# hvasbath/beat

Measured on AMD Instinct MI355X. Metric: SMC chain-steps/s (FFI seismic gfstacking 400 patches x 64 targets x 4096 samples), higher is better.
Workload: dtype f64; 1 GPU; BASELINE configs[2]: FFI seismic gfstacking, 400 patches x 64 targets x 4096 samples, library (64,400,3,25,4096) f64 = 62.9 GB in HBM, nearest_neighbor, covariance scalar; population SURVEY 8(d): nucleation U over the 20x20 fault, time 0; chains_per_gpu=512, global_chains=512, parallelism=chains sharded over 1 GPU(s), library replicated

## Files before the change

beat_amd/csrc/ctx.cpp:

```cpp
#include "ctx.hpp"

#include <cstdlib>

namespace beatamd {

static thread_local char g_err[1024] = "";

void set_error(const char *fmt, ...)
{
    va_list ap;
    va_start(ap, fmt);
    vsnprintf(g_err, sizeof(g_err), fmt, ap);
    va_end(ap);
}

int DevBuf::reserve(size_t bytes)
{
    if (bytes <= cap) return BEATAMD_OK;
    size_t want = bytes + bytes / 4;
    if (p) {
        BA_HIP(hipDeviceSynchronize());
        BA_HIP(hipFree(p));
        p = nullptr;
        cap = 0;
// ... 127 lines not shown
{
    BA_HIP(hipStreamSynchronize(stream));
    int st = 0;
    BA_HIP(hipMemcpy(&st, d_status, sizeof(int), hipMemcpyDeviceToHost));
    if (st) {
        BA_HIP(hipMemset(d_status, 0, sizeof(int)));
        if (st & ST_INDEX_OOB) {
            set_error("index out of bounds of the GF library "
                      "(duration/starttime outside the library grid)");
            return BEATAMD_EINDEX;
        }
        if (st & ST_BAD_HYPO) {
            set_error("nucleation index outside the patch grid");
            return BEATAMD_EINVAL;
        }
        if (st & ST_BAD_COV) {
            set_error("Sample covariances contains Inf or NaN! Please try reducing the upper and lower bounds "
                      "of hyper parameters!");
            return BEATAMD_EBADCOV;
        }
        if (st & ST_NOT_PSD) {
            set_error("Matrix is not positive definite");
            return BEATAMD_ENOTPSD;
        }
        if (st & ST_LINE_NONFINITE) {
            set_error("trace_density: a sample or an extent that is not finite (or xmax <= xmin)");
            return BEATAMD_EINVAL;
        }
        if (st & ST_LINE_OOB) {
            set_error("Line endpoint outside of given grid (an index above the last cell, or below -32768)");
            return BEATAMD_EOUTSIDE;
        }
        if (st & ST_BAD_SCALE) {
            set_error("PoissonProposal: a step width outside (0, 500] (or NaN): the draws of that parameter are NaN");
            return BEATAMD_EINVAL;
        }
    }
    return BEATAMD_OK;
}

namespace beatamd {

void GfKnobs::read_env()
{
    auto rd = [](const char *name) { const char *e = getenv(name); return e ? atoi(e) : KNOB_UNSET; };
    gf_kernel = rd("BEATAMD_GF_KERNEL"); gs_cg = rd("BEATAMD_GS_CG"); gs_ws = rd("BEATAMD_GS_WS"); gs_dma = rd("BEATAMD_GS_DMA");
    gs_nt = rd("BEATAMD_GS_NT"); ws_map = rd("BEATAMD_WS_MAP"); gs_pair = rd("BEATAMD_GS_PAIR"); gs_nthint = rd("BEATAMD_GS_NTHINT");
    gs_order = rd("BEATAMD_GS_ORDER"); gs_fit = rd("BEATAMD_GS_FIT"); gs_win = rd("BEATAMD_GS_WIN"); gf_tinv = rd("BEATAMD_GF_TINV");
    gs_tune = rd("BEATAMD_GS_TUNE"); gf_order = rd("BEATAMD_GF_ORDER"); gf_cgroup = rd("BEATAMD_GF_CGROUP"); gs_ml = rd("BEATAMD_GS_ML");
    gc_global = rd("BEATAMD_GC_GLOBAL"); gc_sort = rd("BEATAMD_GC_SORT"); gc_keys = rd("BEATAMD_GC_KEYS"); gc_bands = rd("BEATAMD_GC_BANDS"); gr_cap = rd("BEATAMD_GR_CAP");
    gr_pass_alloc = rd("BEATAMD_GR_PASS_ALLOC"); gr_var = rd("BEATAMD_GR_VAR"); sweep_v1 = rd("BEATAMD_SWEEP_V1"); qf_band = rd("BEATAMD_QF_BAND"); qf_fuse = rd("BEATAMD_QF_FUSE"); gf_split = rd("BEATAMD_GF_SPLIT"); gm_wave = rd("BEATAMD_GM_WAVE");
    skip_parked = rd("BEATAMD_SKIP_PARKED");
    td_strip = rd("BEATAMD_TD_STRIP");
}

const GfKnobs &gf_knobs(beatamd_ctx *ctx)
{
    if (ctx->knobs_live) ctx->knobs.read_env();
    return ctx->knobs;
}

}

extern "C" {

const char *beatamd_last_error(void) { return g_err; }

int beatamd_version(void) { return BEATAMD_VERSION; }

int beatamd_ctx_create(int device, beatamd_ctx **out)
{
    BA_CHECK(out != nullptr, BEATAMD_EINVAL, "ctx_create: out is NULL");
    int ndev = 0;
    hipError_t e = hipGetDeviceCount(&ndev);
    if (e != hipSuccess || ndev == 0) {
        (void)hipGetLastError();
        set_error("no HIP device available (%s)", hipGetErrorString(e));
        return BEATAMD_EHIP;
    }
    BA_CHECK(device >= 0 && device < ndev, BEATAMD_EINVAL, "device %d out of range [0,%d)", device,
             ndev);
    BA_HIP(hipSetDevice(device));
    beatamd_ctx *c = new beatamd_ctx();
    c->device = device;
    BA_HIP(hipStreamCreateWithFlags(&c->own_stream, hipStreamNonBlocking));
    c->stream = c->own_stream;
    BA_HIP(hipMalloc((void **)&c->d_status, sizeof(int)));
    BA_HIP(hipMemset(c->d_status, 0, sizeof(int)));
    hipDeviceProp_t prop;
    BA_HIP(hipGetDeviceProperties(&prop, device));
    c->num_cu = prop.multiProcessorCount;
    c->scratch_bufs.resize(SL_COUNT);
    c->knobs.read_env();
    {
        const char *live = getenv("BEATAMD_KNOBS_LIVE");
        c->knobs_live = live && atoi(live) != 0;
    }
    *out = c;
    return BEATAMD_OK;
}

int beatamd_ctx_reload_knobs(beatamd_ctx *c)
{
    BA_CHECK(c != nullptr, BEATAMD_EINVAL, "ctx_reload_knobs: NULL context");
    c->knobs.read_env();
    return BEATAMD_OK;
}

int beatamd_ctx_destroy(beatamd_ctx *c)
{
    if (!c) return BEATAMD_OK;
    (void)hipSetDevice(c->device);
    (void)hipStreamSynchronize(c->stream);
    c->models.clear();
    c->hypers.clear();
    c->wsets.clear();
    c->laps.clear();
    c->geolibs.clear();
    c->seislibs.clear();
    for (auto &s : c->scratch_bufs) s.release();
    for (auto &kv : c->timers)
        for (auto &pr : kv.second.pending) {
            (void)hipEventDestroy(pr.first);
            (void)hipEventDestroy(pr.second);
        }
    for (auto e : c->event_pool) (void)hipEventDestroy(e);
    if (c->d_status) (void)hipFree(c->d_status);
    if (c->h_umax) (void)hipHostFree(c->h_umax);
    if (c->umax_event) (void)hipEventDestroy(c->umax_event);
    if (c->own_stream) (void)hipStreamDestroy(c->own_stream);
    delete c;
    return BEATAMD_OK;
}

int beatamd_ctx_set_stream(beatamd_ctx *c, void *s)
{
    BA_CHECK(c, BEATAMD_EINVAL, "ctx is NULL");
    BA_HIP(hipSetDevice(c->device));
    c->stream = (hipStream_t)s;
    return BEATAMD_OK;
}

int beatamd_ctx_use_own_stream(beatamd_ctx *c)
{
    BA_CHECK(c, BEATAMD_EINVAL, "ctx is NULL");
    c->stream = c->own_stream;
    return BEATAMD_OK;
}

int beatamd_ctx_set_step_counter(beatamd_ctx *c, uint32_t *device_counter)
{
    BA_CHECK(c != nullptr, BEATAMD_EINVAL, "ctx is NULL");
    BA_CHECK(device_counter == nullptr || is_device_ptr(device_counter), BEATAMD_EINVAL,
             "ctx_set_step_counter: the counter must live in device memory");
    c->step_dev = device_counter;
    return BEATAMD_OK;
}

int beatamd_ctx_synchronize(beatamd_ctx *c)
{
    BA_CHECK(c, BEATAMD_EINVAL, "ctx is NULL");
    BA_HIP(hipSetDevice(c->device));
    return c->check_status();
}

int beatamd_ctx_enable_timing(beatamd_ctx *c, int on)
{
    BA_CHECK(c, BEATAMD_EINVAL, "ctx is NULL");
    c->timing = on != 0;
    return BEATAMD_OK;
}

static int drain_timer(beatamd_ctx *c, KTimer &t)
{
    for (auto &pr : t.pending) {
        BA_HIP(hipEventSynchronize(pr.second));
        float ms = 0.f;
        BA_HIP(hipEventElapsedTime(&ms, pr.first, pr.second));
        t.total_ms += ms;
        t.n += 1;
        c->event_pool.push_back(pr.first);
        c->event_pool.push_back(pr.second);
// ... 33 lines not shown
```

beat_amd/csrc/ctx.hpp:

```cpp
#pragma once
#include <hip/hip_runtime.h>

#include <cstdarg>
#include <cstdint>
#include <cstdio>
#include <cstring>
#include <map>
#include <memory>
#include <string>
#include <vector>

#include "../../include/beat_amd.h"

struct beatamd_ctx;

namespace beatamd {

void set_error(const char *fmt, ...);

#define BA_HIP(expr)                                                                         \
    do {                                                                                     \
        hipError_t e_ = (expr);                                                              \
        if (e_ != hipSuccess) {                                                              \
            beatamd::set_error("%s:%d: %s -> %s", __FILE__, __LINE__, #expr,                 \
// ... 148 lines not shown
    std::vector<int64_t> sizes;
    std::vector<int32_t> wsets;
    DevMem<int64_t> hp_off;
    bool corr_set = false;
    GeoCorr corr;
    DevMem<GeoCorrTerm> corr_terms;
    DevMem<double> corr_basis;
};

struct GeomSources {
    int nsrc = 0;
    DevMem<int32_t> kind;
    DevMem<int64_t> poff;
    DevMem<double> pfix;
    DevMem<double> east, north, los;
    int64_t Nobs = 0;
    double nu = 0.25;
};

struct FfiModel {
    beatamd_ffi_layout layout;
    int32_t nsub = 0;
    std::vector<int32_t> ndip, nstrike, patch_off;
    std::vector<double> patch_size;
    int64_t P = 0;
    DevMem<int32_t> d_ndip, d_nstrike, d_patch_off;
    DevMem<double> d_patch_size;
    std::vector<Wavemap> wavemaps;
    bool has_geo = false;
    Geodetic geo;
    bool geo_is_geometry = false;
    GeomSources geom;
    int32_t lap = -1;
    int64_t nllk() const;
    bool obs_quads_valid = false;
    std::vector<double> obs_quads;
    DevMem<double> d_obs_quads;
};

struct HyperModel {
    int64_t nterm = 0, nh = 0;
    DevMem<double> M, slog;
    DevMem<int32_t> kind, hp_index;
    int32_t ngroups = 0, group_end[8] = {0, 0, 0, 0, 0, 0, 0, 0};
};

constexpr int KNOB_UNSET = -2147483647;
struct GfKnobs {
    int gf_kernel = KNOB_UNSET, gs_cg = KNOB_UNSET, gs_ws = KNOB_UNSET, gs_dma = KNOB_UNSET, gs_nt = KNOB_UNSET,
        ws_map = KNOB_UNSET, gs_pair = KNOB_UNSET, gs_nthint = KNOB_UNSET, gs_order = KNOB_UNSET, gs_fit = KNOB_UNSET,
        gs_win = KNOB_UNSET, gf_tinv = KNOB_UNSET, gs_tune = KNOB_UNSET, gf_order = KNOB_UNSET, gf_cgroup = KNOB_UNSET,
        gs_ml = KNOB_UNSET, gc_global = KNOB_UNSET, gc_sort = KNOB_UNSET, gc_keys = KNOB_UNSET, gc_bands = KNOB_UNSET, gr_cap = KNOB_UNSET,
        gr_pass_alloc = KNOB_UNSET, gr_var = KNOB_UNSET, sweep_v1 = KNOB_UNSET, qf_band = KNOB_UNSET, qf_fuse = KNOB_UNSET, gf_split = KNOB_UNSET, gm_wave = KNOB_UNSET,
        skip_parked = KNOB_UNSET, td_strip = KNOB_UNSET;
    void read_env();
    static int get(int v, int dflt) { return v == KNOB_UNSET ? dflt : v; }
    static bool is(int v, int x) { return v != KNOB_UNSET && v == x; }
    static bool set(int v) { return v != KNOB_UNSET; }
};

struct KTimer {
    double total_ms = 0;
    int64_t n = 0;
    std::vector<std::pair<hipEvent_t, hipEvent_t>> pending;
};

}

struct beatamd_ctx {
    int device = 0;
    hipStream_t stream = nullptr, own_stream = nullptr;
    bool timing = false;
    std::map<std::string, beatamd::KTimer> timers;
    std::vector<hipEvent_t> event_pool;
    int *d_status = nullptr;
    std::vector<beatamd::DevBuf> scratch_bufs;
    std::vector<std::unique_ptr<beatamd::SeisStore>> seislibs;
    std::vector<std::unique_ptr<beatamd::GeoLib>> geolibs;
    std::vector<std::unique_ptr<beatamd::WeightSet>> wsets;
    std::vector<std::unique_ptr<beatamd::Laplacian>> laps;
    std::vector<std::unique_ptr<beatamd::FfiModel>> models;
    std::vector<std::unique_ptr<beatamd::HyperModel>> hypers;
    int num_cu = 256;
    char last_gf_kernel[96] = "";
    int64_t gs_ngtp = 0, gs_N = 0;
    double gs_trep = 1;
    int gs_nvar = 1;
    bool gs_has_passes = false;
    char gf_plan[384] = "";
    bool gf_band_fused = false;
    char gf_tune_log[512] = "";
    uint32_t *h_umax = nullptr;
    hipEvent_t umax_event = nullptr;
    bool umax_pending = false;
    int umax_hist = -1, umax_hist_cg = 0;
    std::map<std::vector<int64_t>, std::pair<int, int>> gs_tuned;
    int gs_cg = 0;
    beatamd::GfKnobs knobs;
    bool knobs_live = false;
    uint32_t *step_dev = nullptr;

    int get_scratch(int slot, size_t bytes, void **out);
    template <class T>
    int scratch(int slot, size_t n, T **out)
    {
        void *raw = nullptr;
        const int rc = get_scratch(slot, n * sizeof(T), &raw);
        *out = static_cast<T *>(raw);
        return rc;
    }
    hipEvent_t get_event();
    void time_begin(const char *name);
    void time_end(const char *name);
    int check_status();
};

namespace beatamd {

bool is_device_ptr(const void *p);
const GfKnobs &gf_knobs(beatamd_ctx *ctx);

enum Slot : int {
    SL_IN0 = 0, SL_IN1, SL_IN2, SL_IN3, SL_IN4, SL_IN5, SL_IN6, SL_IN7,
    SL_OUT0, SL_OUT1, SL_OUT2, SL_OUT3,
    SL_ROWOFF, SL_WEIGHTS, SL_ST0, SL_RESID, SL_PARTIAL, SL_PARTIAL2, SL_QUAD, SL_MU, SL_SLIPS,
    SL_QPROP, SL_LPROP, SL_MISC, SL_GS_UROWS, SL_GS_UCOUNT, SL_GS_SLOT, SL_GS_W, SL_GS_UMAX, SL_GS_USLOT,
    SL_CHAINBAD, SL_Z, SL_ROWSCALE, SL_CUM, SL_STAGE2, SL_WHITEN,
    SL_CHOL_A, SL_CHOL_X, SL_CHOL_D, SL_CHOL_T, SL_CHOL_L,
    SL_GC_ORDER, SL_GS_ORDER, SL_GC_STREAM, SL_GC_HDR, SL_GC_META, SL_DELTA, SL_LOGU, SL_EDGES, SL_TSLOT, SL_SPLIT, SL_WS_PACK, SL_COUNT
};
constexpr int SL_NIN = SL_OUT0 - SL_IN0, SL_NOUT = SL_ROWOFF - SL_OUT0;

class Staging {
    beatamd_ctx *ctx;
    int nin = 0, nout = 0, nback = 0;
    struct { void *host, *dev; size_t bytes; } back[SL_NOUT];
    int in_bytes(const void *p, size_t bytes, const void **dev);
    int out_bytes(void *p, size_t bytes, void **dev, bool preload);

public:
    explicit Staging(beatamd_ctx *c) : ctx(c) {}
    template <class T>
    int in(const T *p, size_t n, const T **dev)
    {
        const void *d = nullptr;
        BA_TRY(in_bytes(p, n * sizeof(T), &d));
        *dev = static_cast<const T *>(d);
        return BEATAMD_OK;
// ... 21 lines not shown
```

beat_amd/csrc/gfshared.hip:

```cpp
#include "kernels.hpp"

namespace beatamd {

constexpr int GS_NT_MAX = 64;
constexpr int GS_NTHINT_DEFAULT = 1;
constexpr int GS_WS_DEFAULT = 1;

struct GroupTabArgs {
    int nrow, nvar, CG;
    int64_t C, T, P, DS;
    const uint32_t *rowoff;
    const double *fac;
    ChainVec slips[4];
    int ucap, ustride;
    uint32_t *urows;
    uint32_t *uent;
    int nissue;
    int windowed;
    int depth;
    uint32_t *ucount;
    uint32_t *umax;
    uint16_t *slot;
    double *w;
    int64_t w_var_stride;
// ... 1141 lines not shown
            gs_store_syn<GS_NT>(a.out + (c * a.T + t) * N + n0, acc, nvalid);
        }
        return;
    }
    __builtin_amdgcn_s_barrier();
    if (tid < GS_NT) xbuf[tid] = (tid < nvalid) ? a.data[t * N + n0 + tid] : 0.0;
    __builtin_amdgcn_fence(__ATOMIC_RELEASE, "workgroup");
    __builtin_amdgcn_s_barrier();
    __builtin_amdgcn_fence(__ATOMIC_ACQUIRE, "workgroup");
    if (MODE == GF_RESID_STORE) {
        gs_resid_store<GS_NT>(a.out + (c * a.T + t) * N + n0, acc, xbuf, live, nvalid);
    } else {
        const double q = gs_misfit_scalar<GS_NT>(a.wscalar[t], acc, xbuf, nvalid);
        if (live) a.partial[(c * a.T + t) * a.ntile + tile] = q;
    }
}


template <int WAVES, int NROW, int MODE>
static int launch_shared_one(dim3 grid, size_t lds, hipStream_t s, const GsArgs &a)
{
    void (*kern)(GsArgs) = nullptr;
    if constexpr (WAVES == 16) {
        kern = k_gfstack_dma<WAVES, NROW, MODE, 32, 1>;
    } else if (a.f32pair) {
        kern = k_gfstack_dmaf<WAVES, NROW, MODE>;
    } else {
        kern = (a.dma == 2 && a.nt == 32) ? k_gfstack_dma<WAVES, NROW, MODE, 32, 1>
             : (a.dma == 2) ? k_gfstack_dma<WAVES, NROW, MODE, 64, 1>
                            : k_gfstack_dma<WAVES, NROW, MODE, 64, 0>;
    }
    if (lds > 64 * 1024)
        BA_HIP(hipFuncSetAttribute((const void *)kern, hipFuncAttributeMaxDynamicSharedMemorySize, (int)lds));
    hipLaunchKernelGGL(kern, grid, dim3(WAVES * 64), lds, s, a);
    return BEATAMD_OK;
}

template <int WAVES, int NROW>
static int launch_shared_mode(int mode, dim3 grid, size_t lds, hipStream_t s, const GsArgs &a)
{
    if (mode == GF_STORE_SYN) return launch_shared_one<WAVES, NROW, GF_STORE_SYN>(grid, lds, s, a);
    if (mode == GF_RESID_SCALAR) return launch_shared_one<WAVES, NROW, GF_RESID_SCALAR>(grid, lds, s, a);
    return launch_shared_one<WAVES, NROW, GF_RESID_STORE>(grid, lds, s, a);
}

template <int WAVES>
static int launch_shared_nrow(int nrow, int mode, dim3 grid, size_t lds, hipStream_t s,
                              const GsArgs &a)
{
    if (nrow == 1) return launch_shared_mode<WAVES, 1>(mode, grid, lds, s, a);
    return launch_shared_mode<WAVES, 4>(mode, grid, lds, s, a);
}

static int launch_ws(int mode, dim3 grid, size_t lds, hipStream_t s, const GsArgs &a, int pair)
{
    void (*kern)(GsArgs);
#define BA_WS_PICK(NAME, ...)                                                                          \
    (mode == GF_STORE_SYN ? NAME<__VA_ARGS__ GF_STORE_SYN, 3, 1>                                      \
     : mode == GF_RESID_SCALAR ? NAME<__VA_ARGS__ GF_RESID_SCALAR, 3, 1> : NAME<__VA_ARGS__ GF_RESID_STORE, 3, 1>)
#define BA_WS_PICK0(NAME, ...)                                                                         \
    (mode == GF_STORE_SYN ? NAME<__VA_ARGS__ GF_STORE_SYN, 3, 0>                                      \
     : mode == GF_RESID_SCALAR ? NAME<__VA_ARGS__ GF_RESID_SCALAR, 3, 0> : NAME<__VA_ARGS__ GF_RESID_STORE, 3, 0>)
    if (pair == 1) kern = a.nthint ? BA_WS_PICK(k_gfstack_wsp, 1,) : BA_WS_PICK0(k_gfstack_wsp, 1,);
    else if (pair == 2) kern = a.nthint ? BA_WS_PICK(k_gfstack_wsp, 0,) : BA_WS_PICK0(k_gfstack_wsp, 0,);
    else if (mode == GF_RESID_BAND1) kern = a.nthint ? k_gfstack_ws<1, GF_RESID_BAND1, 3, 1> : k_gfstack_ws<1, GF_RESID_BAND1, 3, 0>;
    else kern = a.nthint ? BA_WS_PICK(k_gfstack_ws, 1,) : BA_WS_PICK0(k_gfstack_ws, 1,);
#undef BA_WS_PICK0
#undef BA_WS_PICK
    BA_HIP(hipFuncSetAttribute((const void *)kern, hipFuncAttributeMaxDynamicSharedMemorySize, (int)lds));
    hipLaunchKernelGGL(kern, grid, dim3(768), lds, s, a);
    return BEATAMD_OK;
}

constexpr int WS_CG = 512;
constexpr int WS_LW = 4;
constexpr int WS_USTRIDE = 128;
constexpr int WS_CAP_MAX = 96;
constexpr int WS_MAXPASS = (WS_CG + WS_CAP_MAX - 1) / WS_CAP_MAX;
static bool ws_wanted(const GfStackCall &k, int CG);

struct WsTabArgs {
    int nvar, cap;
    int64_t C, T, P, DS;
    int64_t vmax;
    const uint32_t *rowoff;
    ChainVec slips[4];
    const uint32_t *order;
    uint32_t *npass;
    const uint32_t *voff;
    uint32_t *utotal;
    uint32_t *ucount;
    uint32_t *uent;
    uint16_t *slot;
    double *w;
    int64_t w_var_stride;
    int64_t R;
};

__global__ void __launch_bounds__(256) k_ws_scan(const uint32_t *npass, uint32_t *voff, uint32_t *nv, int64_t P)
{
    __shared__ uint32_t part[256];
    const int tid = threadIdx.x;
    const int64_t gt = blockIdx.x;
    uint32_t run = 0;
    for (int64_t base = 0; base < P; base += 256) {
        const int64_t p = base + tid;
        const uint32_t x = p < P ? npass[gt * P + p] : 0u;
        part[tid] = x;
        __syncthreads();
        uint32_t before = 0, total = 0;
        for (int k = 0; k < 256; k++) {
            const uint32_t y = part[k];
            if (k < tid) before += y;
            total += y;
        }
        if (p < P) voff[gt * P + p] = run + before;
        run += total;
        __syncthreads();
    }
    if (tid == 0) nv[gt] = run;
}

__global__ void __launch_bounds__(WS_CG) k_ws_pack(const uint32_t *order, const int32_t *active, int64_t C, uint32_t *out)
{
    __shared__ uint32_t wsum[WS_CG / 64];
    const int tid = threadIdx.x;
    const int lane = tid & 63, wv = tid >> 6;
    const int64_t pos = (int64_t)blockIdx.x * WS_CG + tid;
    const uint32_t c = order ? order[pos] : (pos < C ? (uint32_t)pos : 0xffffffffu);
    const bool on = c != 0xffffffffu && (int64_t)c < C && active[c] != 0;
    const uint64_t m = __ballot(on);
    if (lane == 0) wsum[wv] = (uint32_t)__popcll(m);
    __syncthreads();
    uint32_t before = 0, total = 0;
    for (int q = 0; q < WS_CG / 64; q++) {
        const uint32_t x = wsum[q];
        if (q < wv) before += x;
        total += x;
    }
    uint32_t *o = out + (int64_t)blockIdx.x * WS_CG;
    if (on) o[before + (uint32_t)__popcll(m & ((1ull << lane) - 1ull))] = c;
    if ((uint32_t)tid >= total) o[tid] = 0xffffffffu;
}
// ... 44 lines not shown
            __syncthreads();
            uint32_t before = 0, total = 0;
            for (int q = 0; q < WS_CG / 64; q++) {
                const uint32_t x = wsum[q];
                if (q < wv) before += x;
                total += x;
            }
            if (f) {
                const uint32_t ps = run + before + (uint32_t)__popcll(m & ((1ull << lane) - 1ull));
                rowmap[i] = (uint16_t)ps;
                if constexpr (FILL) lst[ps] = row0 + (uint32_t)i;
            }
            run += total;
            __syncthreads();
        }
        U = run;
        if (live) pos = rowmap[v - row0];
    } else {
        vals[tid] = v;
        __syncthreads();
        first = live;
        {
            const uint4 *v4 = reinterpret_cast<const uint4 *>(vals);
            for (int k4 = 0; k4 < WS_CG / 4; k4++) {
                const uint4 x = v4[k4];
                const int k = 4 * k4;
                first = first && !((x.x == v && k < tid) || (x.y == v && k + 1 < tid) || (x.z == v && k + 2 < tid) ||
                                   (x.w == v && k + 3 < tid));
            }
        }
        firstv[tid] = first ? v : 0xffffffffu;
        {
            const uint64_t m = __ballot(first);
            if (lane == 0) wsum[wv] = (uint32_t)__popcll(m);
        }
        __syncthreads();
        if (live) {
            const uint4 *f4 = reinterpret_cast<const uint4 *>(firstv);
            for (int k4 = 0; k4 < WS_CG / 4; k4++) {
                const uint4 x = f4[k4];
                pos += (x.x < v) + (x.y < v) + (x.z < v) + (x.w < v);
            }
        }
        for (int q = 0; q < WS_CG / 64; q++) U += wsum[q];
    }
    const int npass = U == 0 ? 1 : (int)((U + (uint32_t)a.cap - 1) / (uint32_t)a.cap);
    if constexpr (!FILL) {
        if (tid == 0) {
            a.npass[gtp] = (uint32_t)npass;
            a.utotal[gtp] = U;
        }
        return;
    }
    if (tid == 0) a.utotal[gtp] = U;
    const int per = U == 0 ? 1 : ((int)U + npass - 1) / npass;
    if constexpr (!MAP) {
        if (first) lst[pos] = v;
    }
    if (live) atomicOr(&gm[pos], 1u << (tid >> 5));
    __syncthreads();
    const int mypass = live ? (int)pos / per : -1;
    if (wv < npass) {
        const int base = wv * per;
        const int n = min(per, (int)U - base);
        if (n <= 32) {
            if (lane < n) slt[base + lane] = (uint16_t)lane;
        } else {
            const int depth = a.cap / 32;
            const int r0 = lane, r1 = lane + 64;
            const uint32_t m0 = r0 < n ? gm[base + r0] : 0u, m1 = r1 < n ? gm[base + r1] : 0u;
            const int key0 = r0 < n ? ((__popc(m0) << 8) | (255 - r0)) : -1;
            const int key1 = r1 < n ? ((__popc(m1) << 8) | (255 - r1)) : -1;
            int rank0 = 0, rank1 = 0;
            for (int j = 0; j < n; j++) {
                const int kj = (__popc(gm[base + j]) << 8) | (255 - j);
                rank0 += kj > key0;
                rank1 += kj > key1;
            }
            if (r0 < n && rank0 < 32) slt[base + r0] = (uint16_t)rank0;
            if (r1 < n && rank1 < 32) slt[base + r1] = (uint16_t)rank1;
            if (r0 < n) rk2i[wv][rank0] = (uint8_t)r0;
            if (r1 < n) rk2i[wv][rank1] = (uint8_t)r1;
            wave_lds_fence();
            uint32_t wmask = 0;
            int wcnt = 0;
            if (lane < 32) {
                wmask = gm[base + rk2i[wv][lane]];
                wcnt = 1;
            }
            for (int rk = 32; rk < n; rk++) {
                const int ridx = (int)rk2i[wv][rk];
                const uint32_t mm = gm[base + ridx];
                int cost = (lane < 32 && wcnt < depth) ? ((__popc(wmask & mm) << 12) | (wcnt << 6) | lane) : 0x7fffffff;
#pragma unroll
                for (int off = 32; off > 0; off >>= 1) cost = min(cost, __shfl_xor(cost, off, 64));
                const int w = cost & 63;
                if (lane == w) {
                    slt[base + ridx] = (uint16_t)(w + 32 * wcnt);
                    wmask |= mm;
                    wcnt++;
                }
            }
        }
    }
    __syncthreads();
    const int64_t v0 = gt * a.vmax + (a.voff ? (int64_t)a.voff[gtp] : p);
    const uint16_t myslot = live ? slt[pos] : (uint16_t)0;
// ... 82 lines not shown

static bool ws_wanted(const GfStackCall &k, int CG)
{
    const GfKnobs &kn = *k.knobs;
    const bool want = GfKnobs::get(kn.gs_ws, GS_WS_DEFAULT) != 0;
    return want && CG == WS_CG && k.interp != BEATAMD_MULTILINEAR && k.libs[0]->N % 2 == 0 &&
           !(GfKnobs::set(kn.gs_dma) && kn.gs_dma != 2) && !(GfKnobs::set(kn.gs_nt) && kn.gs_nt != 64);
}

static void gs_common_args(GsArgs &a, const GfStackCall &k, int64_t Ttab, int64_t ngroups, bool *f32)
{
    const GfKnobs &kn = *k.knobs;
    const SeisLib &L = *k.libs[0];
    memset(&a, 0, sizeof(a));
    *f32 = k.f32;
    for (int v = 0; v < k.nvar; v++) {
        a.G[v] = k.libs[v]->g;
        a.G32[v] = k.libs[v]->g32;
        *f32 = *f32 && a.G32[v] != nullptr;
    }
    a.nvar = k.nvar;
    a.C = k.C; a.T = L.T; a.P = L.P; a.N = L.N;
    a.Ttab = Ttab; a.rows_per_target = L.P * L.D * L.S;
    a.tslot = k.tslot;
    a.ngroups = ngroups;
    a.data = k.data; a.wscalar = k.wscalar; a.out = k.out;
    a.nthint = GfKnobs::set(kn.gs_nthint) ? (kn.gs_nthint != 0) : (GS_NTHINT_DEFAULT && ngroups == 1);
}

static int64_t gs_grid(GsArgs &a, const GfKnobs &kn)
{
    a.xcd_order = (a.ngroups > 1 && !GfKnobs::is(kn.gs_order, 0)) ? 1 : 0;
    if (GfKnobs::is(kn.gs_order, 1)) a.xcd_order = 1;
    return a.xcd_order ? ((a.T * a.ntile + 7) / 8) * 8 * a.ngroups : a.ngroups * a.T * a.ntile;
}

static void gs_record_stats(beatamd_ctx *ctx, const GfStackCall &k, int64_t GTP, int64_t Ttab, int cg, bool has_passes)
{
    ctx->gs_ngtp = GTP;
    ctx->gs_trep = (double)k.libs[0]->T / (double)Ttab;
    ctx->gs_N = k.libs[0]->N;
    ctx->gs_cg = cg;
    ctx->gs_nvar = k.nvar;
    ctx->gs_has_passes = has_passes;
}

static int launch_gfstack_ws(beatamd_ctx *ctx, const GfStackCall &k, const uint32_t *rowoff, int64_t Ttab)
{
    const GfKnobs &kn = *k.knobs;
    const SeisLib &L = *k.libs[0];
    const int64_t ngroups = (k.C + WS_CG - 1) / WS_CG;
    const int64_t GT = ngroups * Ttab, GTP = GT * L.P;
    const int64_t bound = std::min<int64_t>(WS_CG, L.D * L.S);
    const int cap = bound <= 32 ? 32 : bound <= 64 ? 64 : WS_CAP_MAX;
    const int maxpass = (int)((bound + cap - 1) / cap);
    const int64_t vmax = L.P * maxpass;

    WsTabArgs ta;
    memset(&ta, 0, sizeof(ta));
    ta.nvar = k.nvar; ta.cap = cap;
    ta.C = k.C; ta.T = Ttab; ta.P = L.P; ta.DS = L.D * L.S; ta.vmax = vmax;
    ta.rowoff = rowoff;
    for (int v = 0; v < k.nvar; v++) ta.slips[v] = k.slips[v];
    ta.R = k.patch_split;
    if (ngroups > 1 && k.order_key[0].base && k.order_key[1].base && GfKnobs::get(kn.gc_global, 1) != 0)
        BA_TRY(launch_chain_members(ctx, k.C, k.order_key, WS_CG, ngroups, &ta.order, GfKnobs::get(kn.gc_global, 1) == 2));
    BA_TRY(ctx->scratch(SL_GS_UCOUNT, (size_t)(3 * GTP + GT), &ta.utotal));
    ta.npass = ta.utotal + GTP;
    uint32_t *voff = ta.npass + GTP, *nv = voff + GTP;
    const size_t nvs = (size_t)GT * vmax + 3;
    BA_TRY(ctx->scratch(SL_GS_UROWS, nvs, &ta.ucount));
    BA_TRY(ctx->scratch(SL_GS_USLOT, nvs * WS_USTRIDE * 2, &ta.uent));
    BA_TRY(ctx->scratch(SL_GS_SLOT, nvs * WS_CG, &ta.slot));
    ta.w_var_stride = (int64_t)GT * vmax * WS_CG;
    BA_TRY(ctx->scratch(SL_GS_W, (size_t)ta.w_var_stride * k.nvar + (size_t)3 * WS_CG, &ta.w));
    {
        ScopedTimer tm(ctx, "grouptables");
        if (k.active) {
            uint32_t *packed;
            BA_TRY(ctx->scratch(SL_WS_PACK, (size_t)ngroups * WS_CG, &packed));
            hipLaunchKernelGGL(k_ws_pack, dim3((unsigned)ngroups), dim3(WS_CG), 0, ctx->stream, ta.order, k.active, k.C, packed);
            ta.order = packed;
        }
        const bool map = ta.DS <= WS_MAP_MAX && !GfKnobs::is(kn.ws_map, 0);
        const size_t mlds = map ? (size_t)ta.DS * sizeof(uint16_t) : 0;
        if (maxpass > 1) {
            if (map) hipLaunchKernelGGL((k_ws_tables<0, 1>), dim3((unsigned)GTP), dim3(WS_CG), mlds, ctx->stream, ta);
            else hipLaunchKernelGGL((k_ws_tables<0, 0>), dim3((unsigned)GTP), dim3(WS_CG), 0, ctx->stream, ta);
            hipLaunchKernelGGL(k_ws_scan, dim3((unsigned)GT), dim3(256), 0, ctx->stream, ta.npass, voff, nv, L.P);
            ta.voff = voff;
        }
        if (map) hipLaunchKernelGGL((k_ws_tables<1, 1>), dim3((unsigned)GTP), dim3(WS_CG), mlds, ctx->stream, ta);
        else hipLaunchKernelGGL((k_ws_tables<1, 0>), dim3((unsigned)GTP), dim3(WS_CG), 0, ctx->stream, ta);
    }
    BA_HIP(hipGetLastError());

    GsArgs a;
    bool f32;
    gs_common_args(a, k, Ttab, ngroups, &f32);
    const bool pair64 = GfKnobs::is(kn.gs_pair, 1);
    a.nrow = 1;
    a.CG = WS_CG; a.ucap = cap; a.ustride = WS_USTRIDE;
    a.nt = 64; a.dma = 2; a.ws = 3;
    a.ntile = (int)((L.N + 63) / 64);
    a.nv = maxpass > 1 ? nv : nullptr;
    a.vmax = vmax;
    a.order = ta.order;
    a.uent = ta.uent; a.ucount = ta.ucount; a.slot = ta.slot; a.w = ta.w;
    a.w_var_stride = ta.w_var_stride;
    if (k.mode == GF_RESID_SCALAR || k.mode == GF_RESID_BAND1) {
        BA_TRY(ctx->scratch(SL_PARTIAL, (size_t)k.C * L.T * a.ntile, &a.partial));
    }
    if (k.mode == GF_RESID_BAND1) {
        BA_TRY(ctx->scratch(SL_EDGES, (size_t)k.C * L.T * a.ntile * 2, &a.edges));
        a.band_w = k.band_w;
    }
    const int64_t nblocks = gs_grid(a, kn);
    BA_CHECK(nblocks < (int64_t)0x7fffffff, BEATAMD_EINVAL, "gfstack: batch too large");
    size_t lds = f32 ? (size_t)(cap + 1) * (64 + 2) * sizeof(float) * 3
                     : (size_t)(cap + 1) * (64 + (pair64 ? 2 : 1)) * sizeof(double) * 3;
    lds = std::max<size_t>(lds, (64 + 8 * 64 * 17) * sizeof(double));
    BA_CHECK(lds <= 160 * 1024, BEATAMD_EINVAL, "internal: k_gfstack_ws row buffers exceed LDS");
    if (f32 || pair64)
        snprintf(ctx->last_gf_kernel, sizeof(ctx->last_gf_kernel), "k_gfstack_ws%s<%d,%d,%d>", f32 ? "32" : "p64", k.mode, a.ws,
                 a.nthint);
    else
        snprintf(ctx->last_gf_kernel, sizeof(ctx->last_gf_kernel), "k_gfstack_ws<%d,%d,%d,%d>", 1, k.mode, a.ws, a.nthint);
    snprintf(ctx->gf_plan, sizeof(ctx->gf_plan),
             "loader/consumer kernel: 512-chain groups, nearest neighbour; %d row slots per LDS buffer (a patch can touch min(512, "
             "D*S = %lld) rows), %s", cap, (long long)(L.D * L.S),
             maxpass > 1 ? "patches that touch more are staged in passes of equal size" : "one pass per patch");
    gs_record_stats(ctx, k, GTP, Ttab, WS_CG, maxpass > 1);
    {
        ScopedTimer tm(ctx, "gfstack");
        BA_TRY(launch_ws(k.mode, dim3((unsigned)nblocks), lds, ctx->stream, a, f32 ? 1 : (pair64 ? 2 : 0)));
    }
    BA_HIP(hipGetLastError());
    if (k.mode == GF_RESID_SCALAR) BA_TRY(launch_sum_tiles(ctx, a.partial, k.C * L.T, a.ntile, k.quad));
    if (k.mode == GF_RESID_BAND1)
        BA_TRY(launch_sum_tiles_band1(ctx, a.partial, a.edges, k.band_w, k.C, L.T, L.N, a.ntile, 64, k.quad));
    return BEATAMD_OK;
}

int launch_gfstack_shared(beatamd_ctx *ctx, const GfStackCall &k_in, const uint32_t *rowoff,
                          const double *fac, int CG, int ucap, int64_t Ttab)
{
    GfStackCall k = k_in;
    if (k.mode == GF_RESID_BAND1) {
        const GfKnobs &kn0 = *k.knobs;
        bool f32 = k.f32;
        for (int v = 0; v < k.nvar; v++) f32 = f32 && k.libs[v]->g32 != nullptr;
        const bool fuse = ws_wanted(k, CG) && !f32 && !GfKnobs::is(kn0.gs_pair, 1) && !GfKnobs::is(kn0.qf_fuse, 0);
        if (!fuse) k.mode = GF_RESID_STORE;
        ctx->gf_band_fused = fuse;
    }
    if (ws_wanted(k, CG)) return launch_gfstack_ws(ctx, k, rowoff, Ttab);
    const GfKnobs &kn = *k.knobs;
    const SeisLib &L = *k.libs[0];
    const int nrow = k.interp == BEATAMD_MULTILINEAR ? 4 : 1;
    const int64_t ngroups = (k.C + CG - 1) / CG;
    const int64_t GTP = ngroups * Ttab * L.P;

    GroupTabArgs ga;
    memset(&ga, 0, sizeof(ga));
    ga.nrow = nrow; ga.nvar = k.nvar; ga.CG = CG;
    ga.C = k.C; ga.T = Ttab; ga.P = L.P; ga.DS = L.D * L.S;
    ga.rowoff = rowoff; ga.fac = fac;
    for (int v = 0; v < k.nvar; v++) ga.slips[v] = k.slips[v];
    ga.ucap = ucap;
    ga.ustride = (ucap + 63) / 64 * 64;
    BA_TRY(ctx->scratch(SL_GS_UROWS, (size_t)GTP * ga.ustride, &ga.urows));
    BA_TRY(ctx->scratch(SL_GS_USLOT, (size_t)GTP * ga.ustride * 2, &ga.uent));
    BA_TRY(ctx->scratch(SL_GS_UCOUNT, (size_t)GTP, &ga.ucount));
    BA_TRY(ctx->scratch(SL_GS_SLOT, (size_t)(GTP + 3) * nrow * CG, &ga.slot));
    ga.w_var_stride = (nrow == 1) ? ngroups * L.P * CG : GTP * 4 * CG;
    BA_TRY(ctx->scratch(SL_GS_W, (size_t)ga.w_var_stride * k.nvar + (size_t)3 * 4 * CG, &ga.w));
    const bool fit_lds = CG <= 128 && !GfKnobs::is(kn.gs_fit, 0);
    ga.umax = nullptr;
    if (fit_lds) {
        BA_TRY(ctx->scratch(SL_GS_UMAX, 1, &ga.umax));
        BA_HIP(hipMemsetAsync(ga.umax, 0, sizeof(uint32_t), ctx->stream));
    }
    ga.nissue = CG / 64;
    {
        const int depth = (ucap + 31) / 32;
        const bool dma2 = !(GfKnobs::is(kn.gs_dma, 0) || GfKnobs::is(kn.gs_dma, 1)) && L.N % 2 == 0;
        ga.windowed = (CG >= 512 && nrow == 1 && dma2 && ucap > 32 && ucap <= 128 && !GfKnobs::is(kn.gs_win, 0) &&
                       (size_t)2 * 32 * depth * (GS_NT_MAX + 2) * 8 <= 158 * 1024) ? 1 : 0;
// ... 103 lines not shown
```

beat_amd/engine.py:

```python
import ctypes as C

import numpy as np

from . import _lib
from ._lib import INTERPOLATIONS, check, f64, ptr


def _is_dev(a):
    return hasattr(a, "data_ptr") and not isinstance(a, np.ndarray) and a.is_cuda


def _empty_like(ref, shape, dtype=np.float64):
    if _is_dev(ref):
        import torch
        tdt = {np.float64: torch.float64, np.int32: torch.int32}[dtype]
        return torch.empty(shape, dtype=tdt, device=ref.device)
    return np.empty(shape, dtype=dtype)


def _i32(a, ref=None):
    if _is_dev(a):
        import torch
        if a.dtype != torch.int32 or not a.is_contiguous():
            raise ValueError("device index tensors must be contiguous int32")
        return a
    return np.ascontiguousarray(a, dtype=np.int32)


def _i64arr(a):
    return None if a is None else np.ascontiguousarray(a, dtype=np.int64)


def _interp(interpolation):
    if interpolation not in INTERPOLATIONS:
        raise NotImplementedError("Interpolation scheme %s not implemented!" % interpolation)
    return INTERPOLATIONS[interpolation]


class Context(object):

    def __init__(self, device=0):
        self._lib = _lib.load()
        h = C.c_void_p()
        check(self._lib.beatamd_ctx_create(int(device), C.byref(h)))
        self._h = h
        self.device = int(device)

    def close(self):
        if getattr(self, "_h", None):
            self._lib.beatamd_ctx_destroy(self._h)
            self._h = None

    def __del__(self):
# ... 313 lines not shown
            accepted = _empty_like(Q0, (Cn,), np.int32)
        for a in (Q0, L0):
            if isinstance(a, np.ndarray) and not (a.flags.c_contiguous and a.dtype == np.float64):
                raise ValueError("Q0 / L0 must be C-contiguous float64 (updated in place)")
        de, sc, lo, up, lu = f64(delta), f64(scaling), f64(lower), f64(upper), f64(log_u)
        if np.ndim(beta) == 0 and not hasattr(beta, "data_ptr"):
            check(self._lib.beatamd_ffi_astep_batch(self._h, model_id, Cn, ptr(Q0), ptr(L0), ptr(de),
                                                    ptr(sc), ptr(lo), ptr(up), ptr(lu), float(beta),
                                                    ptr(accepted)))
        else:
            be = f64(beta)
            check(self._lib.beatamd_ffi_astep_batch_betas(self._h, model_id, Cn, ptr(Q0), ptr(L0),
                                                          ptr(de), ptr(sc), ptr(lo), ptr(up), ptr(lu),
                                                          ptr(be), ptr(accepted)))
        return accepted

    def ffi_mstep_batch(self, model_id, Q0, L0, factor, kind, df, seed, step, first_chain, scaling, lower,
                        upper, beta, accepted, accepted_sum=None, n_accepted=None):
        self._adopt_stream(Q0, L0)
        Cn = int(Q0.shape[0])
        kind = -1 if kind is None else int(kind)
        fa, sc, lo, up = f64(factor), f64(scaling), f64(lower), f64(upper)
        K = int(fa.shape[0]) if kind < 0 else 0
        scalar = np.ndim(beta) == 0 and not hasattr(beta, "data_ptr")
        be = None if scalar else f64(beta)
        check(self._lib.beatamd_ffi_mstep_batch(
            self._h, model_id, Cn, ptr(Q0), ptr(L0), ptr(fa), K, kind, int(df), int(seed) & (2 ** 64 - 1),
            int(step) & 0xffffffff, int(first_chain), ptr(sc), ptr(lo), ptr(up), float(beta) if scalar else 1.0,
            None if scalar else ptr(be), ptr(accepted), None if accepted_sum is None else ptr(accepted_sum),
            None if n_accepted is None else ptr(n_accepted)))
        return accepted

    def last_kernel(self):
        buf = C.create_string_buffer(128)
        check(self._lib.beatamd_ctx_last_kernel(self._h, buf, 128))
        return buf.value.decode()

    def gf_group_stats(self):
        cg, mx, rb, mean = C.c_int64(), C.c_int64(), C.c_int64(), C.c_double()
        check(self._lib.beatamd_ctx_gf_group_stats(self._h, C.byref(cg), C.byref(mean), C.byref(mx),
                                                   C.byref(rb)))
        return dict(chains_per_group=cg.value, mean_rows=mean.value, max_rows=mx.value,
                    row_bytes=rb.value)

    def reload_knobs(self):
        check(self._lib.beatamd_ctx_reload_knobs(self._h))

    def gf_plan(self, passes=True):
        buf = C.create_string_buffer(512)
        mean, mx = C.c_double(), C.c_int64()
        check(self._lib.beatamd_ctx_gf_plan(self._h, buf, 512, C.byref(mean) if passes else None,
                                            C.byref(mx) if passes else None))
        out = dict(plan=buf.value.decode())
        if passes:
            out.update(mean_passes=mean.value, max_passes=mx.value)
        return out

    def gf_tune_log(self):
        buf = C.create_string_buffer(512)
        check(self._lib.beatamd_ctx_gf_tune_log(self._h, buf, 512))
        return buf.value.decode()

    def gf_chain_groups(self, key0, key1, chains_per_group=512):
        import torch
        dev = "cuda:%d" % self.device
        k0, k1 = [k if _is_dev(k) else torch.as_tensor(np.ascontiguousarray(k, dtype=np.float64)).to(dev) for k in (key0, key1)]
        self._adopt_stream(k0, k1)
        k0, k1 = f64(k0), f64(k1)
        Cn = int(k0.numel())
        ng = (Cn + chains_per_group - 1) // chains_per_group
        out = np.empty(ng * chains_per_group, dtype=np.uint32)
        check(self._lib.beatamd_ctx_gf_chain_groups(self._h, Cn, ptr(k0), ptr(k1), int(chains_per_group),
                                                    out.ctypes.data_as(C.c_void_p)))
        return out.reshape(ng, chains_per_group)

    def smc_calc_beta(self, likelihoods, beta, coef_variation, stride=1, n=None):
        self._adopt_stream(likelihoods)
        lk = f64(likelihoods)
        Cn = int(n if n is not None else (lk.numel() if _is_dev(lk) else lk.size))
        w = _empty_like(lk, (Cn,))
        b = C.c_double()
        check(self._lib.beatamd_smc_calc_beta(self._h, Cn, ptr(lk), int(stride), float(beta),
                                              float(coef_variation), C.byref(b), ptr(w)))
        return b.value, w

    def smc_stage_weights(self, likelihoods, dbeta, stride=1, n=None):
        self._adopt_stream(likelihoods)
        lk = f64(likelihoods)
        Cn = int(n if n is not None else (lk.numel() if _is_dev(lk) else lk.size))
        w = _empty_like(lk, (Cn,))
        check(self._lib.beatamd_smc_stage_weights(self._h, Cn, ptr(lk), int(stride), float(dbeta), ptr(w)))
        return w

    def smc_resample(self, weights, aux):
        self._adopt_stream(weights)
        w = f64(weights)
        Cn = int(w.numel()) if _is_dev(w) else int(w.size)
        idx = _empty_like(w, (Cn,), np.int32)
        check(self._lib.beatamd_smc_resample(self._h, Cn, ptr(w), float(aux), ptr(idx)))
        return idx

    def smc_population_factor(self, population, weights):
        self._adopt_stream(population, weights)
        X, w = f64(population), f64(weights)
        Cn, npar = int(X.shape[0]), int(X.shape[1])
        F = _empty_like(X, (Cn, npar))
# ... 347 lines not shown
```

Before: 92540 chain-steps/s.

## Use four-deep LDS row-buffer ring when patches touch at most 64 rows

Adds a four-buffer ring variant of the loader/consumer gfstack kernel, capping row slots at 64 so four buffers fit in LDS. The choice is made from a device-side atomicMax of the unique-row count per patch, read back asynchronously from the previous launch of the same shape, so there is no synchronous stall. The deeper ring lets loads run further ahead of the consumers. In exchange it uses more LDS per block, and patches that exceed 64 rows may need more passes. The first call of each shape, and calls made under stream capture, keep the three-buffer path.

```diff
diff --git a/beat_amd/csrc/ctx.cpp b/beat_amd/csrc/ctx.cpp
--- a/beat_amd/csrc/ctx.cpp
+++ b/beat_amd/csrc/ctx.cpp
@@ -203,6 +203,7 @@
     gr_pass_alloc = rd("BEATAMD_GR_PASS_ALLOC"); gr_var = rd("BEATAMD_GR_VAR"); sweep_v1 = rd("BEATAMD_SWEEP_V1"); qf_band = rd("BEATAMD_QF_BAND"); qf_fuse = rd("BEATAMD_QF_FUSE"); gf_split = rd("BEATAMD_GF_SPLIT"); gm_wave = rd("BEATAMD_GM_WAVE");
     skip_parked = rd("BEATAMD_SKIP_PARKED");
     td_strip = rd("BEATAMD_TD_STRIP");
+    ws_ring = rd("BEATAMD_WS_RING");
 }
 
 const GfKnobs &gf_knobs(beatamd_ctx *ctx)
@@ -279,6 +280,8 @@
     if (c->d_status) (void)hipFree(c->d_status);
     if (c->h_umax) (void)hipHostFree(c->h_umax);
     if (c->umax_event) (void)hipEventDestroy(c->umax_event);
+    if (c->h_ws_umax) (void)hipHostFree(c->h_ws_umax);
+    if (c->ws_umax_event) (void)hipEventDestroy(c->ws_umax_event);
     if (c->own_stream) (void)hipStreamDestroy(c->own_stream);
     delete c;
     return BEATAMD_OK;
diff --git a/beat_amd/csrc/ctx.hpp b/beat_amd/csrc/ctx.hpp
--- a/beat_amd/csrc/ctx.hpp
+++ b/beat_amd/csrc/ctx.hpp
@@ -224,7 +224,7 @@
         gs_win = KNOB_UNSET, gf_tinv = KNOB_UNSET, gs_tune = KNOB_UNSET, gf_order = KNOB_UNSET, gf_cgroup = KNOB_UNSET,
         gs_ml = KNOB_UNSET, gc_global = KNOB_UNSET, gc_sort = KNOB_UNSET, gc_keys = KNOB_UNSET, gc_bands = KNOB_UNSET, gr_cap = KNOB_UNSET,
         gr_pass_alloc = KNOB_UNSET, gr_var = KNOB_UNSET, sweep_v1 = KNOB_UNSET, qf_band = KNOB_UNSET, qf_fuse = KNOB_UNSET, gf_split = KNOB_UNSET, gm_wave = KNOB_UNSET,
-        skip_parked = KNOB_UNSET, td_strip = KNOB_UNSET;
+        skip_parked = KNOB_UNSET, td_strip = KNOB_UNSET, ws_ring = KNOB_UNSET;
     void read_env();
     static int get(int v, int dflt) { return v == KNOB_UNSET ? dflt : v; }
     static bool is(int v, int x) { return v != KNOB_UNSET && v == x; }
@@ -259,13 +259,18 @@
     double gs_trep = 1;
     int gs_nvar = 1;
     bool gs_has_passes = false;
-    char gf_plan[384] = "";
+    char gf_plan[512] = "";
     bool gf_band_fused = false;
     char gf_tune_log[512] = "";
     uint32_t *h_umax = nullptr;
     hipEvent_t umax_event = nullptr;
     bool umax_pending = false;
     int umax_hist = -1, umax_hist_cg = 0;
+    uint32_t *h_ws_umax = nullptr;
+    hipEvent_t ws_umax_event = nullptr;
+    bool ws_umax_pending = false;
+    int ws_umax_hist = -1;
+    std::vector<int64_t> ws_umax_key, ws_umax_pending_key;
     std::map<std::vector<int64_t>, std::pair<int, int>> gs_tuned;
     int gs_cg = 0;
     beatamd::GfKnobs knobs;
diff --git a/beat_amd/csrc/gfshared.hip b/beat_amd/csrc/gfshared.hip
--- a/beat_amd/csrc/gfshared.hip
+++ b/beat_amd/csrc/gfshared.hip
@@ -1217,19 +1217,22 @@
     return launch_shared_mode<WAVES, 4>(mode, grid, lds, s, a);
 }
 
-static int launch_ws(int mode, dim3 grid, size_t lds, hipStream_t s, const GsArgs &a, int pair)
+static int launch_ws(int mode, dim3 grid, size_t lds, hipStream_t s, const GsArgs &a, int pair, int nb)
 {
     void (*kern)(GsArgs);
-#define BA_WS_PICK(NAME, ...)                                                                          \
-    (mode == GF_STORE_SYN ? NAME<__VA_ARGS__ GF_STORE_SYN, 3, 1>                                      \
-     : mode == GF_RESID_SCALAR ? NAME<__VA_ARGS__ GF_RESID_SCALAR, 3, 1> : NAME<__VA_ARGS__ GF_RESID_STORE, 3, 1>)
-#define BA_WS_PICK0(NAME, ...)                                                                         \
-    (mode == GF_STORE_SYN ? NAME<__VA_ARGS__ GF_STORE_SYN, 3, 0>                                      \
-     : mode == GF_RESID_SCALAR ? NAME<__VA_ARGS__ GF_RESID_SCALAR, 3, 0> : NAME<__VA_ARGS__ GF_RESID_STORE, 3, 0>)
-    if (pair == 1) kern = a.nthint ? BA_WS_PICK(k_gfstack_wsp, 1,) : BA_WS_PICK0(k_gfstack_wsp, 1,);
-    else if (pair == 2) kern = a.nthint ? BA_WS_PICK(k_gfstack_wsp, 0,) : BA_WS_PICK0(k_gfstack_wsp, 0,);
+#define BA_WS_PICK(NAME, NB_, ...)                                                                     \
+    (mode == GF_STORE_SYN ? NAME<__VA_ARGS__ GF_STORE_SYN, NB_, 1>                                    \
+     : mode == GF_RESID_SCALAR ? NAME<__VA_ARGS__ GF_RESID_SCALAR, NB_, 1> : NAME<__VA_ARGS__ GF_RESID_STORE, NB_, 1>)
+#define BA_WS_PICK0(NAME, NB_, ...)                                                                    \
+    (mode == GF_STORE_SYN ? NAME<__VA_ARGS__ GF_STORE_SYN, NB_, 0>                                    \
+     : mode == GF_RESID_SCALAR ? NAME<__VA_ARGS__ GF_RESID_SCALAR, NB_, 0> : NAME<__VA_ARGS__ GF_RESID_STORE, NB_, 0>)
+    BA_CHECK(nb == 3 || (nb == 4 && pair == 0), BEATAMD_EINVAL, "internal: k_gfstack_ws has rings of three or four row buffers");
+    if (pair == 1) kern = a.nthint ? BA_WS_PICK(k_gfstack_wsp, 3, 1,) : BA_WS_PICK0(k_gfstack_wsp, 3, 1,);
+    else if (pair == 2) kern = a.nthint ? BA_WS_PICK(k_gfstack_wsp, 3, 0,) : BA_WS_PICK0(k_gfstack_wsp, 3, 0,);
+    else if (nb == 4 && mode == GF_RESID_BAND1) kern = a.nthint ? k_gfstack_ws<1, GF_RESID_BAND1, 4, 1> : k_gfstack_ws<1, GF_RESID_BAND1, 4, 0>;
+    else if (nb == 4) kern = a.nthint ? BA_WS_PICK(k_gfstack_ws, 4, 1,) : BA_WS_PICK0(k_gfstack_ws, 4, 1,);
     else if (mode == GF_RESID_BAND1) kern = a.nthint ? k_gfstack_ws<1, GF_RESID_BAND1, 3, 1> : k_gfstack_ws<1, GF_RESID_BAND1, 3, 0>;
-    else kern = a.nthint ? BA_WS_PICK(k_gfstack_ws, 1,) : BA_WS_PICK0(k_gfstack_ws, 1,);
+    else kern = a.nthint ? BA_WS_PICK(k_gfstack_ws, 3, 1,) : BA_WS_PICK0(k_gfstack_ws, 3, 1,);
 #undef BA_WS_PICK0
 #undef BA_WS_PICK
     BA_HIP(hipFuncSetAttribute((const void *)kern, hipFuncAttributeMaxDynamicSharedMemorySize, (int)lds));
@@ -1241,7 +1244,9 @@
 constexpr int WS_LW = 4;
 constexpr int WS_USTRIDE = 128;
 constexpr int WS_CAP_MAX = 96;
-constexpr int WS_MAXPASS = (WS_CG + WS_CAP_MAX - 1) / WS_CAP_MAX;
+constexpr int WS_CAP_RING4 = 64;
+constexpr int WS_MAXPASS = WS_CG / WS_CAP_RING4;
+static_assert(WS_MAXPASS == WS_CG / 64, "k_ws_tables: one of its wavefronts per pass");
 static bool ws_wanted(const GfStackCall &k, int CG);
 
 struct WsTabArgs {
@@ -1254,6 +1259,7 @@
     uint32_t *npass;
     const uint32_t *voff;
     uint32_t *utotal;
+    uint32_t *umax;
     uint32_t *ucount;
     uint32_t *uent;
     uint16_t *slot;
@@ -1404,7 +1410,10 @@
         }
         return;
     }
-    if (tid == 0) a.utotal[gtp] = U;
+    if (tid == 0) {
+        a.utotal[gtp] = U;
+        if (a.umax) atomicMax(a.umax, U);
+    }
     const int per = U == 0 ? 1 : ((int)U + npass - 1) / npass;
     if constexpr (!MAP) {
         if (first) lst[pos] = v;
@@ -1593,7 +1602,49 @@
     const int64_t ngroups = (k.C + WS_CG - 1) / WS_CG;
     const int64_t GT = ngroups * Ttab, GTP = GT * L.P;
     const int64_t bound = std::min<int64_t>(WS_CG, L.D * L.S);
-    const int cap = bound <= 32 ? 32 : bound <= 64 ? 64 : WS_CAP_MAX;
+    bool f32_ring = k.f32;
+    for (int v = 0; v < k.nvar; v++) f32_ring = f32_ring && k.libs[v]->g32 != nullptr;
+    const bool ring_fixed = f32_ring || GfKnobs::is(kn.gs_pair, 1) || GfKnobs::is(kn.ws_ring, 3);
+    int nb = 3;
+    const char *ring_why = "BEATAMD_WS_RING";
+    bool post_count = false;
+    if (ring_fixed) {
+        if (!GfKnobs::is(kn.ws_ring, 3)) ring_why = "pair gather";
+    } else if (GfKnobs::is(kn.ws_ring, 4)) {
+        nb = 4;
+    } else if (bound <= WS_CAP_RING4) {
+        nb = 4;
+        ring_why = "a patch cannot touch more rows";
+    } else {
+        hipStreamCaptureStatus cs = hipStreamCaptureStatusNone;
+        BA_HIP(hipStreamIsCapturing(ctx->stream, &cs));
+        if (cs != hipStreamCaptureStatusNone) {
+            ring_why = "stream capture";
+        } else {
+            const std::vector<int64_t> key = {k.C, L.T, L.P, L.N, L.D * L.S, (int64_t)k.nvar, Ttab, (int64_t)k.patch_split};
+            if (!ctx->h_ws_umax) {
+                BA_HIP(hipHostMalloc((void **)&ctx->h_ws_umax, sizeof(uint32_t), hipHostMallocDefault));
+                BA_HIP(hipEventCreateWithFlags(&ctx->ws_umax_event, hipEventDisableTiming));
+            }
+            if (ctx->ws_umax_pending && hipEventQuery(ctx->ws_umax_event) == hipSuccess) {
+                ctx->ws_umax_hist = (int)*ctx->h_ws_umax;
+                ctx->ws_umax_key = ctx->ws_umax_pending_key;
+                ctx->ws_umax_pending = false;
+            }
+            (void)hipGetLastError();
+            if (ctx->ws_umax_hist >= 0 && ctx->ws_umax_key == key) {
+                if (ctx->ws_umax_hist <= WS_CAP_RING4) nb = 4;
+                ring_why = nb == 4 ? "previous launch: at most 64 rows per patch" : "previous launch: more than 64 rows in a patch";
+            } else {
+                ring_why = "no earlier launch of this shape";
+            }
+            if (!ctx->ws_umax_pending) {
+                post_count = true;
+                ctx->ws_umax_pending_key = key;
+            }
+        }
+    }
+    const int cap = bound <= 32 ? 32 : (bound <= 64 || nb == 4) ? WS_CAP_RING4 : WS_CAP_MAX;
     const int maxpass = (int)((bound + cap - 1) / cap);
     const int64_t vmax = L.P * maxpass;
 
@@ -1604,6 +1655,10 @@
     ta.rowoff = rowoff;
     for (int v = 0; v < k.nvar; v++) ta.slips[v] = k.slips[v];
     ta.R = k.patch_split;
+    if (post_count) {
+        BA_TRY(ctx->scratch(SL_GS_UMAX, 1, &ta.umax));
+        BA_HIP(hipMemsetAsync(ta.umax, 0, sizeof(uint32_t), ctx->stream));
+    }
     if (ngroups > 1 && k.order_key[0].base && k.order_key[1].base && GfKnobs::get(kn.gc_global, 1) != 0)
         BA_TRY(launch_chain_members(ctx, k.C, k.order_key, WS_CG, ngroups, &ta.order, GfKnobs::get(kn.gc_global, 1) == 2));
     BA_TRY(ctx->scratch(SL_GS_UCOUNT, (size_t)(3 * GTP + GT), &ta.utotal));
@@ -1635,6 +1690,11 @@
         else hipLaunchKernelGGL((k_ws_tables<1, 0>), dim3((unsigned)GTP), dim3(WS_CG), 0, ctx->stream, ta);
     }
     BA_HIP(hipGetLastError());
+    if (post_count) {
+        BA_HIP(hipMemcpyAsync(ctx->h_ws_umax, ta.umax, sizeof(uint32_t), hipMemcpyDeviceToHost, ctx->stream));
+        BA_HIP(hipEventRecord(ctx->ws_umax_event, ctx->stream));
+        ctx->ws_umax_pending = true;
+    }
 
     GsArgs a;
     bool f32;
@@ -1658,8 +1718,9 @@
     }
     const int64_t nblocks = gs_grid(a, kn);
     BA_CHECK(nblocks < (int64_t)0x7fffffff, BEATAMD_EINVAL, "gfstack: batch too large");
+    BA_CHECK(nb == 3 || !(f32 || pair64), BEATAMD_EINVAL, "internal: the pair gathers have a ring of three row buffers");
     size_t lds = f32 ? (size_t)(cap + 1) * (64 + 2) * sizeof(float) * 3
-                     : (size_t)(cap + 1) * (64 + (pair64 ? 2 : 1)) * sizeof(double) * 3;
+                     : (size_t)(cap + 1) * (64 + (pair64 ? 2 : 1)) * sizeof(double) * (size_t)nb;
     lds = std::max<size_t>(lds, (64 + 8 * 64 * 17) * sizeof(double));
     BA_CHECK(lds <= 160 * 1024, BEATAMD_EINVAL, "internal: k_gfstack_ws row buffers exceed LDS");
     if (f32 || pair64)
@@ -1668,13 +1729,13 @@
     else
         snprintf(ctx->last_gf_kernel, sizeof(ctx->last_gf_kernel), "k_gfstack_ws<%d,%d,%d,%d>", 1, k.mode, a.ws, a.nthint);
     snprintf(ctx->gf_plan, sizeof(ctx->gf_plan),
-             "loader/consumer kernel: 512-chain groups, nearest neighbour; %d row slots per LDS buffer (a patch can touch min(512, "
-             "D*S = %lld) rows), %s", cap, (long long)(L.D * L.S),
+             "loader/consumer kernel: 512-chain groups, nearest neighbour; ring of %d LDS buffers of %d row slots (%s; a patch can "
+             "touch min(512, D*S = %lld) rows), %s", nb, cap, ring_why, (long long)(L.D * L.S),
              maxpass > 1 ? "patches that touch more are staged in passes of equal size" : "one pass per patch");
     gs_record_stats(ctx, k, GTP, Ttab, WS_CG, maxpass > 1);
     {
         ScopedTimer tm(ctx, "gfstack");
-        BA_TRY(launch_ws(k.mode, dim3((unsigned)nblocks), lds, ctx->stream, a, f32 ? 1 : (pair64 ? 2 : 0)));
+        BA_TRY(launch_ws(k.mode, dim3((unsigned)nblocks), lds, ctx->stream, a, f32 ? 1 : (pair64 ? 2 : 0), nb));
     }
     BA_HIP(hipGetLastError());
     if (k.mode == GF_RESID_SCALAR) BA_TRY(launch_sum_tiles(ctx, a.partial, k.C * L.T, a.ntile, k.quad));
diff --git a/beat_amd/engine.py b/beat_amd/engine.py
--- a/beat_amd/engine.py
+++ b/beat_amd/engine.py
@@ -1,4 +1,5 @@
 import ctypes as C
+import re
 
 import numpy as np
 
@@ -418,6 +419,8 @@
         check(self._lib.beatamd_ctx_gf_plan(self._h, buf, 512, C.byref(mean) if passes else None,
                                             C.byref(mx) if passes else None))
         out = dict(plan=buf.value.decode())
+        ring = re.search(r"ring of (\d+) LDS buffers of (\d+) row slots", out["plan"])
+        out.update(ring_buffers=int(ring.group(1)) if ring else 0, ring_slots=int(ring.group(2)) if ring else 0)
         if passes:
             out.update(mean_passes=mean.value, max_passes=mx.value)
         return out
```

After: 91480 chain-steps/s. -1.1%, worse.
